# ryought/dbgphmm

Hardware: AMD Instinct MI355X
Metric: read-bases/sec through forward+backward P(R|X) (higher is better)
Workload: dtype f64; 1 GPU; cfg3: synthetic 100 kb diploid genome (1% divergence), 20x HiFi reads (p=0.001, L=1000), k=40 DBG; sparse-adaptive forward+backward+posteriors (generate_mappings); n_nodes=131694, n_edges=132357, reads_rank0=4026, bases_rank0=4000713, total_bases=4000713, spin_up_steps=12

## Files before the change

dbgphmm_amd/csrc/api.cpp:

```cpp
#include <chrono>
#include <cstdlib>
#include <cmath>
#include <cstring>

#include "phmm_internal.h"

namespace phmm {

static thread_local std::string g_error;
static thread_local hipStream_t g_stream = nullptr;
static thread_local uint64_t g_ws_limit = 0;
static thread_local CallStats g_stats;
static thread_local bool g_timing = false;

void set_error(const std::string &msg) { g_error = msg; }
int fail(int code, const std::string &msg) {
    g_error = msg;
    return code;
}
hipStream_t current_stream() { return g_stream; }
int &workset_index() {
    static thread_local int idx = 0;
    return idx;
}
// ... 40 lines not shown
    k.no_packed = flag("PHMM_NO_PACKED");
    k.packed_cpl = num("PHMM_PACKED_CPL", 0);
    k.no_exact_hinted = flag("PHMM_NO_EXACT_HINTED");
    k.no_exact_dense = flag("PHMM_NO_EXACT_DENSE");
    k.no_wide_hinted = flag("PHMM_NO_WIDE_HINTED");
    k.wide_hinted = flag("PHMM_WIDE_HINTED") && !k.no_wide_hinted;
    k.no_wide_list_bwd = flag("PHMM_NO_WIDE_LIST_BWD");
    k.wide_edge_bwd = flag("PHMM_WIDE_EDGE_BWD");
    k.wide_states_bwd = flag("PHMM_WIDE_STATES_BWD");
    k.wide_bwd_t = num("PHMM_WIDE_BWD_T", 0);
    if (k.wide_bwd_t != 128 && k.wide_bwd_t != 448) k.wide_bwd_t = 0;
    k.wide_hinted_cpb = num("PHMM_WIDE_HINTED_CPB", 0);
    if (k.wide_hinted_cpb != 1 && k.wide_hinted_cpb != 2 && k.wide_hinted_cpb != 4) k.wide_hinted_cpb = 0;
    k.no_side_worker = flag("PHMM_NO_SIDE_WORKER");
    k.no_wide_handover = flag("PHMM_NO_WIDE_HANDOVER");
    k.workers = std::max(1, std::min(MAX_WORKERS, num("PHMM_WORKERS", 1)));
    k.warm_cols = num("PHMM_WARM_COLS", 0);
    k.chunk_groups = std::max(0, num("PHMM_CHUNK_GROUPS", 0));
    k.no_keep_all = flag("PHMM_NO_KEEP_ALL");
    k.pipeline_min_groups = std::max(1, num("PHMM_PIPELINE_MIN_GROUPS", 8));
    k.no_runmax = flag("PHMM_NO_RUNMAX");
    k.force_radix = flag("PHMM_FORCE_RADIX");
    k.no_bwd_skip = flag("PHMM_NO_BWD_SKIP");
    k.serial_emit = flag("PHMM_SERIAL_EMIT");
    k.emit_high_priority = flag("PHMM_EMIT_HIGH_PRIORITY");
    k.no_dma = flag("PHMM_NO_DMA");
    k.bwd_dma = flag("PHMM_BWD_DMA");
    k.dense_streams = num("PHMM_DENSE_STREAMS", 0);
    k.dense_w = num("PHMM_DENSE_W", 0);
    k.dense_npt = num("PHMM_DENSE_NPT", 0);
    if (const char *e = std::getenv("PHMM_MEM_FRACTION")) k.mem_fraction = std::min(0.97, std::max(0.1, std::atof(e)));
    k.share_prefix = num("PHMM_SHARE_PREFIX", -1);
    if (k.share_prefix < 0 || k.share_prefix > 6) k.share_prefix = -1;
    g_knobs = k;
}

void trace(const char *tag) {
    if (!g_knobs.trace) return;
    static thread_local std::chrono::steady_clock::time_point last = std::chrono::steady_clock::now();
    (void)hipStreamSynchronize(g_stream);
    const auto now = std::chrono::steady_clock::now();
    static const auto t0 = std::chrono::steady_clock::now();
    std::fprintf(stderr, "[phmm trace] w%d @%9.2f %-28s %8.2f ms\n", workset_index(),
                 std::chrono::duration<double, std::milli>(now - t0).count(), tag,
                 std::chrono::duration<double, std::milli>(now - last).count());
    last = now;
}

uint64_t table_budget(const DevicePool &pool, uint64_t reserve) {
    if (g_ws_limit) return g_ws_limit;
    size_t fr = 0, tot = 0;
    if (hipMemGetInfo(&fr, &tot) != hipSuccess) return (uint64_t)16 << 30;
    const double frac = g_knobs.mem_fraction > 0.0 ? g_knobs.mem_fraction : 0.9;
    const double b = frac * (double)(fr + pool.owned_table_bytes()) - (double)reserve;
    return (uint64_t)std::max(b, 64.0 * 1024 * 1024);
}
uint64_t planned_budget(const DevicePool &pool) {
    if (g_ws_limit) return g_ws_limit;
    size_t fr = 0, tot = 0;
    if (hipMemGetInfo(&fr, &tot) != hipSuccess) return (uint64_t)16 << 30;
    const double frac = g_knobs.mem_fraction > 0.0 ? g_knobs.mem_fraction : 0.95;
    return (uint64_t)(frac * (double)(fr + pool.owned_bytes()));
}

static std::mutex g_pool_mu;
static DevicePool *g_pools[64] = {};
// ... 896 lines not shown
```

dbgphmm_amd/csrc/dense.hip:

```cpp
#include <algorithm>
#include <cmath>
#include <cstring>
#include <numeric>
#include <type_traits>

#include "dense_internal.h"
#include "lds_dma.h"
#include "prefix_share.h"

#ifndef PHMM_FWD_PF
#define PHMM_FWD_PF 2
#endif
#ifndef PHMM_BWD_PF
#define PHMM_BWD_PF 1
#endif
#ifndef PHMM_SMALLW_WAVES
#define PHMM_SMALLW_WAVES 3
#endif

namespace phmm {


__device__ __forceinline__ int xcd_block(int b, int nblk8) {
    int per = nblk8 >> 3;
// ... 481 lines not shown
    const int cn = a.bcols == 2 ? ((pos + 1) & 1) : (pos + 1 < a.Lc ? pos + 1 : 0);
    const int cc = a.bcols == 2 ? (pos & 1) : pos;
    const double *nm = a.Bm + ((size_t)g * a.bcols + cn) * NW;
    const double *ni = a.Bi + ((size_t)g * a.bcols + cn) * NW;
    double *om = a.Bm + ((size_t)g * a.bcols + cc) * NW;
    double *oi = a.Bi + ((size_t)g * a.bcols + cc) * NW;
    double *od = a.Bd ? a.Bd + ((size_t)g * a.bcols + cc) * NW : nullptr;

    double wgt = 0.0, wgt2 = 0.0;
    const double *fm = nullptr, *fi = nullptr, *fd = nullptr, *gm = nullptr, *gi = nullptr, *gd = nullptr;
    const bool want_post = a.want_freq || a.want_map;
    if (want_post && live) {
        const double lpf = a.logPf[g * W + r];
        if (lpf > -INFINITY) {
            if (pos >= 1) {
                const int fe = a.FE[((size_t)g * (a.Lc + 1) + (pos - 1)) * W + r];
                wgt = exp((double)(fe + Epos) * LN2 - lpf);
            }
            if (first && !sparse_tail) {
                const int fe = a.FE[((size_t)g * (a.Lc + 1) + pos) * W + r];
                wgt2 = exp((double)fe * LN2 - lpf) * lp.p_end;
            }
        }
    }
    if (want_post) {
        const size_t cprev = ((size_t)g * a.Lc + (pos > 0 ? pos - 1 : 0)) * NW;
        const size_t ccur = ((size_t)g * a.Lc + pos) * NW;
        fm = a.Fm + cprev; fi = a.Fi + cprev; fd = a.Fd + cprev;
        gm = a.Fm + ccur; gi = a.Fi + ccur; gd = a.Fd + ccur;
    }
    int rf = r;
    if (VF && want_post) {
        const uint32_t v = share_lane_of_column(a.vlane[g * W + r], pos - 1);
        const size_t vc = ((size_t)(v / SHARE_W) * a.vLc + (pos - 1)) * NW;
        fm = a.vFm + vc; fi = a.vFi + vc; fd = a.vFd + vc;
        rf = (int)(v % SHARE_W);
    }

    double vmax = 0.0, s1 = 0.0, s2 = 0.0, pmx = 0.0, pmx2 = 0.0;
    double *Pa = a.want_map ? a.Pa + (size_t)g * NW : nullptr;
    double *Pb = a.want_map ? a.Pb + (size_t)g * NW : nullptr;
    if (lb < a.nblk && compute) {
        constexpr int H = CHAIN_HOPS;
        const int kbase = lb * (a.npt * ROWS) + row * a.npt + hull_first;
        double E1 = 0.0, E2 = 0.0, E3 = 0.0, E4 = 0.0, E5 = 0.0, Q1 = 0.0, Q2 = 0.0, Q3 = 0.0, Q4 = 0.0, Q5 = 0.0, TE = 0.0;
        int nvalid = 0;
        constexpr int PFB = DMA_ ? BDMA_DEPTH : PHMM_BWD_PF;
        double nx_m[PFB], nx_i[PFB], nx_fm[PFB], nx_fi[PFB], nx_fd[PFB];
        const double *lfm = want_post ? fm : nm, *lfi = want_post ? fi : nm, *lfd = want_post ? fd : nm;
        const int jtop = hull_top < a.N - 1 - kbase ? hull_top : a.N - 1 - kbase;
        const int l64 = threadIdx.x & 63;
        const double *srcA = (l64 < 32 ? nm : ni) + 2 * (l64 & 31);
        const double *srcB = (l64 < 32 ? lfm : lfi) + 2 * (l64 & 31);
        const double *srcC = lfd + 2 * (l64 & 31);
        const uint32_t ring_base =
            DMA_ ? (uint32_t)__builtin_amdgcn_readfirstlane(
                       (int)(uint32_t)(uintptr_t)&ring[(threadIdx.x >> 6) * BDMA_DEPTH * BDMA_SLOT])
                 : 0u;
        const double *ring_w = &ring[DMA_ ? (threadIdx.x >> 6) * BDMA_DEPTH * BDMA_SLOT : 0];
        const int n1 = __any(live) ? 2 + (od ? 1 : 0) : 0;
        if (W == 64 && a.skcells) {
            const unsigned long long nlive = (unsigned long long)__popcll(__ballot(live));
            if (l64 == 0 && jtop >= 0) atomicAdd(a.skcells, nlive * (unsigned long long)(jtop + 1));
        }
        const int ns = n1 + ((a.want_map && __any(live)) ? 1 : 0) + (a.want_freq ? 2 : 0);
#pragma unroll
        for (int u = 0; u < PFB; u++) {
            int v0 = kbase + (jtop - u > 0 ? jtop - u : 0);
// ... 960 lines not shown
```

dbgphmm_amd/csrc/dense_internal.h:

```cpp
#pragma once

#include <vector>

#include "phmm_internal.h"
#include "seg_hull.h"

namespace phmm {

static constexpr double LN2 = 0.693147180559945309417232121458;
static constexpr int BLOCK = 256;

struct DenseArgs {
    int N, ng, Lc, nblk, npt;
    int g_off;
    const NodeRec *nodes;
    const uint8_t *emis;
    const double *init, *dinit, *tdinit;
    const uint32_t *fc_off;
    const FwdEntry *fc;
    const uint32_t *bc_off;
    const BwdEntry *bc;
    const uint32_t *fh_off, *bh_off;
    const HopEntry *fh, *bh;
    int hop_mode;
// ... 6 lines not shown
    unsigned long long *cmaxF;
    double *epart;
    int eall;
    double *logPf;
    double *logE;
    double *Bm, *Bi, *Bd;
    int bcols;
    int *BE;
    unsigned long long *cmaxB;
    double *bpart;
    double *logmbB, *logibB;
    double *accg;
    int want_freq;
    int nblk8;
    unsigned long long *tmaxF;
    const int *bstart;
    int want_map;
    double *Pa, *Pb;
    double *Prun;
    unsigned long long *pmax;
    const int *wf_sw;
    const uint8_t *wf_mode;
    int *wf_sub;
    int *wf_cnt;
    uint32_t *wf_node;
    double *wf_tot;
    double wf_ratio;
    double wf_ub_a, wf_ub_b;
    const uint32_t *rs_off = nullptr, *rs = nullptr;
    uint32_t *skH = nullptr;
    uint8_t *skA = nullptr;
    int nrun = 0, nseg = 0, sseg = 1;
    unsigned long long *skcells = nullptr;
    const double *vFm = nullptr, *vFi = nullptr, *vFd = nullptr;
    const uint32_t *vlane = nullptr;
    int vLc = 0, vJ = 0;
};
static constexpr int WF_CAP = 1024;


struct Plan {
    int W, ng_total, npt, nblk, nblk8;
    std::vector<uint32_t> order;
};

Plan make_plan(const phmm_model *m, const phmm_reads *reads, int forced_w);
Plan make_plan_ids(const phmm_model *m, const phmm_reads *reads, const std::vector<uint32_t> &ids);
void layout(DenseArgs &a, int W, bool full_b, void *tables, void *misc, size_t &tb, size_t &mb,
            bool backward_only = false);
void fill_model_args(DenseArgs &a, const phmm_model *m);
void host_logib(const phmm_model *m, size_t n, std::vector<double> &out);
void launch_fwd_step(int W, const DenseArgs &a, int pos);
void launch_fwd_finish(int W, const DenseArgs &a);
void launch_bwd_step(int W, const DenseArgs &a, int pos);
void launch_bwd_finish(int W, const DenseArgs &a);

struct ExactTables {
    double *f_m, *f_i, *f_d, *f_scal, *b_m, *b_i, *b_d, *b_scal;
};
void exact_dense_reads(phmm_model *m, const uint8_t *bases, const uint64_t *off, const std::vector<uint32_t> &ids, double *lf,
                       double *lb, double *freq_dev, const ExactTables *tabs, double *edge_freq_dev = nullptr,
                       double *init_freq_dev = nullptr);
bool certify_dense(int N, int len, double log2P, const int *FE, const double *log2maxF, const int *BE, const double *log2maxB,
                   double log2_p_end);
bool certify_dense_cells(int N, int len, const int *E, const double *log2max, bool backward);

}
// ... 1 lines not shown
```

dbgphmm_amd/csrc/phmm_internal.h:

```cpp
#pragma once

#include <hip/hip_runtime.h>

#include <cstdint>
#include <cstdio>
#include <memory>
#include <mutex>
#include <string>
#include <vector>

#include "../../include/phmm_amd.h"
#include "../../include/phmm_amd_states.h"
#include "../../include/phmm_amd_path.h"
#include "../../include/phmm_amd_share.h"

namespace phmm {

void set_error(const std::string &msg);
int fail(int code, const std::string &msg);

struct Error {
    int code;
    std::string msg;
};
// ... 311 lines not shown
    bool trace = false;
    bool no_lean = false;
    bool no_wide_class = false;
    bool no_packed = false;
    int packed_cpl = 0;
    bool no_exact_hinted = false;
    bool no_exact_dense = false;
    bool wide_hinted = false;
    bool no_wide_hinted = false;
    bool no_wide_list_bwd = false;
    bool wide_edge_bwd = false;
    bool wide_states_bwd = false;
    int wide_bwd_t = 0;
    int wide_hinted_cpb = 0;
    bool no_side_worker = false;
    bool no_wide_handover = false;
    int workers = 1;
    int warm_cols = 0;
    int chunk_groups = 0;
    bool no_keep_all = false;
    int pipeline_min_groups = 8;
    bool no_runmax = false;
    bool force_radix = false;
    bool serial_emit = false;
    bool emit_high_priority = false;
    bool no_dma = false;
    bool bwd_dma = false;
    bool no_bwd_skip = false;
    int dense_streams = 0;
    int dense_w = 0;
    int dense_npt = 0;
    double mem_fraction = 0.0;
    int share_prefix = -1;
};
const Knobs &knobs();
void refresh_knobs();

void model_build_host(phmm_model *m);
void model_upload(phmm_model *m);
const RunSucc &model_run_successors(phmm_model *m, int seg);

void run_dense(phmm_model *m, const phmm_reads *reads, double *out_lf, double *out_lb,
               double *out_nf);
void full_prob_sparse_backward(phmm_model *m, const phmm_reads *reads, double *out_logp, double *out_total);
void backward_sparse_tables(phmm_model *m, const uint8_t *read, uint64_t len, double *b_m, double *b_i, double *b_d,
                            double *b_scal, uint8_t *is_dense);
void run_sparse(phmm_model *m, const phmm_reads *reads, double *out_lf, double *out_lb, double *out_nf);
void run_dense_edges(phmm_model *m, const phmm_reads *reads, double *out_lf, double *out_ef, double *out_if);
struct RecPool;
void full_prob_reads_hinted(phmm_model *m, const phmm_reads *reads, const phmm_mappings *mp, uint32_t n_cand,
                            const double *init_logp, const double *trans_logp, double *out_logp,
                            double *out_total, const RecPool *pool = nullptr, const uint32_t *copy_nums = nullptr,
                            uint32_t min_copy_num = 0);
void full_prob_reads_copy_num_changes(phmm_model *m, const phmm_reads *reads, const phmm_mappings *mp,
                                      const uint32_t *base_cn, uint32_t min_cn, uint32_t n_cand, const uint64_t *chg_off,
                                      const uint32_t *chg_node, const uint32_t *chg_cn, double *out_logp,
                                      double *out_total, uint64_t *out_n_rescored);
void likelihood_refresh(phmm_likelihood *lk);
void likelihood_score_changes(phmm_likelihood *lk, uint32_t n_cand, const uint64_t *chg_off, const uint32_t *chg_node,
                              const uint32_t *chg_cn, double *out_logp, double *out_total, uint64_t *out_n_rescored,
                              bool by_group = false);
void likelihood_move(phmm_likelihood *lk, uint64_t n_chg, const uint32_t *chg_node, const uint32_t *chg_cn,
                     double *out_total, uint64_t *out_n_rescored, bool by_group = false);
void likelihood_current(const phmm_likelihood *lk, uint32_t *out_cn, double *out_logp, double *out_total);
void upload_reads(const phmm_reads *r);
void upload_mappings(const phmm_mappings *mp);
// ... 24 lines not shown
```

dbgphmm_amd/csrc/prefix_share.h:

```cpp
#pragma once

#include <cstdint>

#if defined(__HIPCC__)
#define PHMM_SHARE_FN __host__ __device__ inline
#else
#define PHMM_SHARE_FN inline
#endif

namespace phmm {

static constexpr int SHARE_MIN_J = 2, SHARE_MAX_J = 6;
static constexpr int SHARE_W = 64;
static constexpr uint64_t SHARE_MEM_DIV = 16;

PHMM_SHARE_FN uint32_t share_lanes(int J) { return 1u << (2 * J); }
PHMM_SHARE_FN uint32_t share_groups(int J) { return (share_lanes(J) + SHARE_W - 1) / SHARE_W; }
PHMM_SHARE_FN uint64_t share_table_bytes(int J, uint64_t N) {
    return (uint64_t)share_groups(J) * (uint64_t)J * N * SHARE_W * 24;
}

PHMM_SHARE_FN int64_t share_gain(int ng, int J) { return (int64_t)ng * J - (int64_t)J * (int64_t)share_groups(J); }

PHMM_SHARE_FN int share_choose_j(int ng, uint64_t N, uint64_t cap) {
    int best = 0;
    int64_t best_gain = 0;
    for (int J = SHARE_MIN_J; J <= SHARE_MAX_J; J++) {
        if (share_table_bytes(J, N) > cap) break;
        const int64_t g = share_gain(ng, J);
        if (g > best_gain) {
            best = J;
            best_gain = g;
        }
    }
    return best;
}

PHMM_SHARE_FN uint32_t share_prefix_index(const uint8_t *digit, int J) {
    uint32_t idx = 0;
    for (int i = 0; i < J; i++) idx |= (uint32_t)(digit[i] & 3u) << (2 * i);
    return idx;
}
PHMM_SHARE_FN uint32_t share_digit(uint32_t idx, int i) { return (idx >> (2 * i)) & 3u; }
PHMM_SHARE_FN uint32_t share_lane_of_column(uint32_t idx, int j) { return idx & (share_lanes(j + 1) - 1u); }

}
```

dbgphmm_amd/csrc/sparse_dyn.hip:

```cpp
#include <algorithm>
#include <cmath>
#include <cstdlib>
#include <cstring>

#include "dense_internal.h"
#include <condition_variable>
#include <deque>
#include <exception>
#include <functional>
#include <memory>
#include <mutex>
#include <thread>

#include "frontier_dev.h"
#include "prefix_share.h"
#include "sparse_dyn.h"
#include "sparse_fwd_kernel.h"
#include "wide_fwd_kernel.h"
#include "lean_fwd_kernel.h"

namespace phmm {

struct WarmArgs {
    DenseArgs d;
// ... 159 lines not shown
    if (lane == 0) {
        if (decided) {
            wa.sw[gi] = new_sw;
            if (new_sw < len) wa.cand_n[gi] = new_cn;
        }
        wa.amb[gi] = amb ? 1 : 0;
        if (amb) atomicAdd(wa.n_amb, 1);
        else if (!decided) atomicAdd(wa.undecided, 1);
        ((uint8_t *)wa.d.wf_mode)[gi] = (!decided && pos >= 1 && nsub <= 4096) ? 1 : 0;
        wa.d.wf_sub[gi] = 0;
        wa.d.wf_cnt[gi] = 0;
    }
}

struct ShareArgs {
    DenseArgs v;
    DenseArgs d;
    const uint32_t *vlane;
    int J;
};
__global__ void __launch_bounds__(BLOCK) share_copy_ctl(const ShareArgs sa, const int lanes) {
    const int gi = blockIdx.x * BLOCK + threadIdx.x;
    if (gi >= lanes || sa.d.len[gi] == 0) return;
    const int g = gi / SHARE_W, r = gi % SHARE_W;
    const uint32_t idx = sa.vlane[gi];
    for (int j = 0; j < sa.J; j++) {
        const uint32_t v = share_lane_of_column(idx, j);
        const size_t vg = v / SHARE_W, vr = v % SHARE_W;
        sa.d.FE[((size_t)g * (sa.d.Lc + 1) + j) * SHARE_W + r] = sa.v.FE[(vg * (sa.v.Lc + 1) + j) * SHARE_W + vr];
        sa.d.cmaxF[((size_t)g * sa.d.Lc + j) * SHARE_W + r] = sa.v.cmaxF[(vg * sa.v.Lc + j) * SHARE_W + vr];
        if (j + 1 < sa.J) sa.d.tmaxF[((size_t)g * sa.d.Lc + j) * SHARE_W + r] = sa.v.tmaxF[(vg * sa.v.Lc + j) * SHARE_W + vr];
    }
}
static constexpr int SHARE_ROWS = 32;
__global__ void __launch_bounds__(BLOCK) share_expand(const ShareArgs sa, const int nrange) {
    const unsigned b = blockIdx.x;
    const unsigned t = b >> 3;
    const int g = (int)(t % (unsigned)sa.d.ng);
    const int c = (int)(t / (unsigned)sa.d.ng) * 8 + (int)(b & 7u);
    if (c >= nrange) return;
    const int r = threadIdx.x & 63, w = threadIdx.x >> 6;
    const int gi = g * SHARE_W + r;
    const bool on = sa.d.len[gi] != 0;
    const uint32_t v = sa.vlane[gi];
    const size_t NW = (size_t)sa.d.N * SHARE_W;
    const size_t so = ((size_t)(v / SHARE_W) * sa.v.Lc + (sa.J - 1)) * NW + v % SHARE_W;
    const size_t dof = ((size_t)g * sa.d.Lc + (sa.J - 1)) * NW + r;
    const double *sm = sa.v.Fm + so, *si = sa.v.Fi + so;
    double *dm = sa.d.Fm + dof, *di = sa.d.Fi + dof;
    constexpr int PER = SHARE_ROWS / (BLOCK / 64);
    double vm[PER], vi[PER];
    const int k0 = c * SHARE_ROWS + w;
#pragma unroll
    for (int u = 0; u < PER; u++) {
        const int k = k0 + u * (BLOCK / 64);
        const bool ok = on && k < sa.d.N;
        vm[u] = ok ? sm[(size_t)k * SHARE_W] : 0.0;
        vi[u] = ok ? si[(size_t)k * SHARE_W] : 0.0;
    }
#pragma unroll
    for (int u = 0; u < PER; u++) {
        const int k = k0 + u * (BLOCK / 64);
        if (on && k < sa.d.N) {
            dm[(size_t)k * SHARE_W] = vm[u];
            di[(size_t)k * SHARE_W] = vi[u];
        }
    }
}

__device__ __forceinline__ int block_count(int local, int *lds_i) {
    __syncthreads();
    if (threadIdx.x == 0) *lds_i = 0;
    __syncthreads();
    local = wave_isum(local);
    if ((threadIdx.x & 63) == 0) atomicAdd(lds_i, local);
    __syncthreads();
    return *lds_i;
}

__global__ void __launch_bounds__(BLOCK) select_top400(const Top400Args a) {
    __shared__ int cnt;
    const uint32_t gi = a.need[blockIdx.x];
    const int g = (int)(gi / a.W), r = (int)(gi % a.W);
    const int col = a.sw[gi] - 1;
    const int N = a.d.N;
    const size_t NW = (size_t)N * a.W;
    const double *fm = a.d.Fm + ((size_t)g * a.d.Lc + col) * NW;
    const double *fi = a.d.Fi + ((size_t)g * a.d.Lc + col) * NW;
    const double *fd = a.d.Fd + ((size_t)g * a.d.Lc + col) * NW;
    const double tmax = __longlong_as_double((long long)a.d.tmaxF[((size_t)g * a.d.Lc + col) * a.W + r]);
    const double thr = tmax * a.ratio_lin;
    uint32_t *sn = a.sc_node + (size_t)blockIdx.x * N;
    double *stt = a.sc_tot + (size_t)blockIdx.x * N;
    if (threadIdx.x == 0) a.sc_n[blockIdx.x] = 0;
    __syncthreads();
    for (int k = threadIdx.x; k < N; k += BLOCK) {
        const size_t ix = (size_t)k * a.W + r;
        const double t = fm[ix] + fi[ix] + fd[ix];
// ... 128 lines not shown
    uint64_t min_len = UINT64_MAX;
    for (uint64_t r = 0; r < R; r++) min_len = std::min<uint64_t>(min_len, reads->off[r + 1] - reads->off[r]);
    const int map_planes = sink ? (min_len <= (uint64_t)prm.n_warmup + 2 ? 3 : 2) : 0;
    uint64_t limit_total = 0, limit_side = 0;
    {
        const uint64_t est_fpool = reads->total * 1024 + R * 65536 + (1u << 20), est_meta = reads->total * 40,
                       est_ctl = R * (uint64_t)(PHMM_MAX_ACTIVE_NODES * 12 * 5 + WF_CAP * 12 + 4096) + reads->total,
                       est_sink = sink ? reads->total * 176 + R * 131072 + (1u << 21) : 0,
                       est_sel = (uint64_t)256 * m->N * 12;
        const uint64_t est = (est_fpool + est_meta + est_ctl) * 5 / 4 + est_sink + est_sel;
        uint64_t have = m->pool->ws_out.bytes;
        for (const auto &w : m->pool->wsets) {
            have += w.misc.bytes;
            for (int k = 0; k < 16; k++)
                if (k != 4) have += w.aux[k].bytes;
        }
        const uint64_t total = planned_budget(*m->pool), fixed = std::max(est, have);
        limit_total = total > fixed + ((uint64_t)64 << 20) ? total - fixed : (uint64_t)64 << 20;
        uint64_t n_def = std::max<uint64_t>(8, R / 50);
        if (by_ratio && reads->warm_hint.size() == R) {
            n_def = 8;
            for (uint16_t h : reads->warm_hint) n_def += h >= warm_cols ? 1 : 0;
        }
        const uint64_t per_read = ((uint64_t)(prm.n_warmup + 2) * 24 + 4 * 8 + (uint64_t)map_planes * 8) * m->N;
        uint64_t lanes_def = 1;
        while (lanes_def < std::min<uint64_t>(n_def, 64)) lanes_def <<= 1;
        if (n_def > 64) lanes_def = (n_def + 63) / 64 * 64;
        limit_side = std::min<uint64_t>(limit_total / 8, lanes_def * per_read * 9 / 8);
    }
    uint64_t limit_main = limit_total - limit_side;

    struct ShareState {
        int J = 0;
        uint32_t nvl = 0;
        DenseArgs va{};
        int digit_of[256];
        double ms = 0.0;
        uint64_t launches = 0, cells = 0;
    } share;
    share_info() = ShareInfo();
    std::vector<uint32_t> short_ids;
    if (by_ratio && main_pc->plan.W == SHARE_W && knobs().share_prefix != 0) {
        const uint64_t cap = limit_main / SHARE_MEM_DIV;
        const int forced = knobs().share_prefix;
        int J = forced > 0 ? (share_table_bytes(forced, m->N) <= cap ? forced : 0)
                           : share_choose_j(main_pc->plan.ng_total, m->N, cap);
        if (J > 0 && (int64_t)J + 2 > prm.n_warmup) J = 0;
        if (J > 0 && min_len < (uint64_t)J + 2) {
            if (forced > 0) J = 0;
            else {
                for (uint64_t r = 0; r < R; r++)
                    if (reads->off[r + 1] - reads->off[r] < (uint64_t)J + 2) short_ids.push_back((uint32_t)r);
                if (short_ids.size() > std::max<uint64_t>(8, R / 50)) J = 0;
                else {
                    std::vector<uint32_t> long_ids;
                    for (uint64_t r = 0; r < R; r++)
                        if (reads->off[r + 1] - reads->off[r] >= (uint64_t)J + 2) long_ids.push_back((uint32_t)r);
                    Plan lp = make_plan_ids(m, reads, long_ids);
                    if (lp.W == SHARE_W) main_pc->plan = std::move(lp);
                    else J = 0;
                }
                if (J == 0) short_ids.clear();
            }
        }
        const auto in_main = [&](uint64_t r) { return short_ids.empty() || reads->off[r + 1] - reads->off[r] >= (uint64_t)J + 2; };
        if (J > 0) {
            std::fill(share.digit_of, share.digit_of + 256, -1);
            bool seen[256] = {};
            for (uint8_t e : m->emission) seen[e] = true;
            int nc = 0;
            for (int b = 0; b < 256; b++)
                if (seen[b] && b != (int)'n') share.digit_of[b] = nc++;
            if (nc > 4) J = 0;
            for (uint64_t r = 0; r < R && J > 0; r++)
                for (int i = 0; i < J && in_main(r); i++)
                    if (share.digit_of[reads->bases[reads->off[r] + i]] < 0) {
                        J = 0;
                        break;
                    }
        }
        if (J > 0) {
            const uint64_t vl = (uint64_t)share_groups(J) * SHARE_W;
            const uint64_t bytes = share_table_bytes(J, m->N) + vl * ((uint64_t)PHMM_MAX_ACTIVE_NODES * 12 + 64 * (J + 1)) +
                                   (uint64_t)share_groups(J) * m->N * 8 + ((uint64_t)4 << 20);
            limit_main -= std::min(bytes, limit_main / 2);
            share.J = J;
            share.nvl = share_lanes(J);
        }
    }

    auto enqueue_plan = [&](std::unique_ptr<PlanCtx> pcu, std::deque<Item> &dst) {
        PlanCtx *pc = pcu.get();
        Plan &plan = pc->plan;
        for (uint32_t rd : plan.order) pc->max_len = std::max<uint64_t>(pc->max_len, reads->off[rd + 1] - reads->off[rd]);
        if (by_ratio && reads->warm_hint.size() == reads->R)
            std::stable_sort(plan.order.begin(), plan.order.end(),
                             [&](uint32_t x, uint32_t y) { return reads->warm_hint[x] > reads->warm_hint[y]; });
        const int W = plan.W;
        const size_t NW = (size_t)m->N * W;
        pc->d_order.upload(plan.order.data(), sizeof(uint32_t) * plan.order.size());
        HIP_CHECK(hipStreamSynchronize(current_stream()));
        int target = chunk_groups;
        if (target == 0) target = n_workers > 1 ? std::max(4, (plan.ng_total + 3 * n_workers - 1) / (3 * n_workers)) : plan.ng_total;
        const uint64_t limit = (&dst == &side_queue) ? limit_side : limit_main / (uint64_t)n_workers;
        int g0 = 0;
        while (g0 < plan.ng_total) {
            int Lc = (int)std::min<int64_t>((int64_t)pc->max_len, std::min<int64_t>(prm.n_warmup + 2, pc->lc_cap));
            if (pc->may_defer && g0 == 0 && n_workers == 1) {
                auto cost = [&](int lc) { return (size_t)lc * NW * 24 + 4 * NW * 8 + (sink ? (size_t)map_planes * NW * 8 + (size_t)plan.nblk8 * BLOCK * 8 : 0); };
                const int lc_full = (int)std::min<int64_t>((int64_t)pc->max_len, prm.n_warmup + 2);
                if ((uint64_t)plan.ng_total * cost(lc_full) <= limit && !knobs().no_keep_all) Lc = lc_full;
                else
                    for (int cut = 0; cut <= 2 && Lc - cut >= 8; cut++)
                        if ((uint64_t)plan.ng_total * cost(Lc - cut) <= limit) {
                            Lc -= cut;
                            break;
                        }
            }
            const size_t per_group = (size_t)Lc * NW * 24 + 4 * NW * 8 + (sink ? (size_t)map_planes * NW * 8 + (size_t)plan.nblk8 * BLOCK * 8 : 0);
            int ngc = (int)std::min<uint64_t>(plan.ng_total - g0, std::max<uint64_t>(1, limit / std::max<size_t>(per_group, 1)));
            ngc = std::min(ngc, std::max(1, target));
            int Lfull = 1;
            for (size_t slot = (size_t)g0 * W; slot < std::min<size_t>(plan.order.size(), (size_t)(g0 + ngc) * W); slot++) {
                const uint32_t rd = plan.order[slot];
                Lfull = std::max(Lfull, (int)(reads->off[rd + 1] - reads->off[rd]));
            }
            dst.push_back(Item{pc, g0, ngc, std::min(Lc, Lfull), Lfull});
            g0 += ngc;
        }
        plans.push_back(std::move(pcu));
    };

    std::function<void()> start_side_worker;
    auto run_chunk = [&](const Item &it) {
        hipStream_t s = current_stream();
        CallStats &st = stats();
        DevBuf &warm = m->wset().aux[0];
        DevBuf &fpool = m->wset().aux[1], &fpool_meta = m->wset().aux[2];
        const Plan &plan = it.pc->plan;
        const DevBuf &d_order = it.pc->d_order;
        const int W = plan.W;
        const uint64_t R = plan.order.size();
        const int g0 = it.g0, ngc = it.ngc, Lc = it.Lc, Lfull = it.Lfull;
// ... 55 lines not shown
        }
        std::vector<double> hib;
        host_logib(m, (size_t)Lc, hib);
        std::vector<int> hlc(hl);
        for (auto &v : hlc) v = std::min(v, Lc);
        {
            StageArgs sa{};
            sa.bases = reads->d_bases.as<uint8_t>();
            sa.off = reads->d_off.as<uint64_t>();
            sa.order = d_order.as<uint32_t>() + (size_t)g0 * W;
            sa.n_slots = (uint32_t)(R - std::min<uint64_t>(R, (uint64_t)g0 * W));
            sa.W = W;
            sa.Lc = Lc;
            sa.Lfull = Lfull;
            sa.out_dense = (uint8_t *)a.bases;
            sa.out_full = (uint8_t *)(wp + o_bases);
            const unsigned per_group = (unsigned)Lfull * W;
            hipLaunchKernelGGL(stage_bases, dim3((per_group + BLOCK - 1) / BLOCK, ngc), dim3(BLOCK), 0, s, sa);
            HIP_CHECK(hipGetLastError());
        }
        HIP_CHECK(hipMemcpyAsync((void *)a.len, hlc.data(), hlc.size() * sizeof(int), hipMemcpyHostToDevice, s));
        HIP_CHECK(hipMemcpyAsync((void *)a.logib, hib.data(), hib.size() * sizeof(double), hipMemcpyHostToDevice, s));
        std::vector<uint32_t> hvl(shared ? (size_t)lanes : 0, 0u);
        if (shared) {
            for (int gi = 0; gi < lanes; gi++) {
                const size_t slot = (size_t)g0 * W + gi;
                if (slot >= R) continue;
                const uint8_t *rb = reads->bases.data() + reads->off[plan.order[slot]];
                uint8_t dg[SHARE_MAX_J];
                for (int i = 0; i < share.J; i++) dg[i] = (uint8_t)share.digit_of[rb[i]];
                hvl[gi] = share_prefix_index(dg, share.J);
            }
            HIP_CHECK(hipMemcpyAsync(wp + o_vlane, hvl.data(), sizeof(uint32_t) * lanes, hipMemcpyHostToDevice, s));
            a.vFm = share.va.Fm;
            a.vFi = share.va.Fi;
            a.vFd = share.va.Fd;
            a.vlane = (const uint32_t *)(wp + o_vlane);
            a.vLc = share.va.Lc;
            a.vJ = share.J;
        }
        HIP_CHECK(hipStreamSynchronize(s));

        WarmArgs wa{};
        wa.d = a;
        wa.sw = (int *)(wp + o_sw);
        wa.cnt = (int *)(wp + o_cnt);
        wa.cand_n = (int *)(wp + o_cn);
        wa.undecided = (int *)(wp + o_und);
        wa.n_amb = wa.undecided + 1;
        wa.amb = (int *)(wp + o_amb);
        a.wf_sw = by_ratio ? wa.sw : nullptr;
        a.wf_mode = (const uint8_t *)(wp + o_mode);
        a.wf_sub = (int *)(wp + o_wsub);
        a.wf_cnt = (int *)(wp + o_wcnt);
        a.wf_node = (uint32_t *)(wp + o_wnode);
        a.wf_tot = (double *)(wp + o_wtot);
        a.wf_ratio = std::exp(-prm.active_node_max_ratio);
        a.wf_ub_a = m->wf_ub_a;
        a.wf_ub_b = m->wf_ub_b;
        wa.d = a;
        wa.cand_node = (uint32_t *)(wp + o_cnode);
        wa.cand_tot = (double *)(wp + o_ctot);
        wa.ratio_lin = std::exp(-prm.active_node_max_ratio);
        wa.n_warmup = (int)prm.n_warmup;
        wa.threshold = (int)prm.warmup_threshold;

        trace("staging+upload");
        int pos = 0;
        const bool st_on = W == 64 && (it.pc->may_defer || !by_ratio);
        LaunchTimer lt(timing_enabled() && st_on);
        std::unique_lock<std::mutex> dense_lock(dense_token, std::defer_lock);
        const bool use_token = it.pc->may_defer || !by_ratio;
        if (use_token) dense_lock.lock();
        if (shared) {
            ShareArgs sa{share.va, a, a.vlane, share.J};
            const int nrange = (int)((m->N + SHARE_ROWS - 1) / SHARE_ROWS), nrange8 = (nrange + 7) / 8 * 8;
            lt.begin();
            hipLaunchKernelGGL(share_copy_ctl, dim3((lanes + BLOCK - 1) / BLOCK), dim3(BLOCK), 0, s, sa, lanes);
            hipLaunchKernelGGL(share_expand, dim3((unsigned)nrange8 * (unsigned)ngc), dim3(BLOCK), 0, s, sa, nrange);
            lt.end();
            HIP_CHECK(hipGetLastError());
            pos = share.J;
        }
        if (!by_ratio) {
            const int last = std::min<int>((int)prm.n_warmup, Lc);
            for (pos = 0; pos <= last; pos++) {
                lt.begin();
                launch_fwd_step(W, a, pos);
                lt.end();
                if (st_on) st.launches[0]++;
            }
            std::vector<int> fsw(lanes);
            for (int gi = 0; gi < lanes; gi++) fsw[gi] = std::min<int>((int)prm.n_warmup, hl[gi]);
            HIP_CHECK(hipMemcpyAsync(wa.sw, fsw.data(), sizeof(int) * lanes, hipMemcpyHostToDevice, s));
            HIP_CHECK(hipStreamSynchronize(s));
        }
        for (; by_ratio; pos++) {
            lt.begin();
            launch_fwd_step(W, a, pos);
            lt.end();
            if (st_on) st.launches[0]++;
            HIP_CHECK(hipMemsetAsync(wa.undecided, 0, sizeof(int) * 2, s));
            hipLaunchKernelGGL(warm_decide_fused, dim3((lanes + BLOCK / 64 - 1) / (BLOCK / 64)), dim3(BLOCK), 0, s, wa, pos,
                               lanes, W);
            int und[2] = {0, 0};
            HIP_CHECK(hipMemcpyAsync(und, wa.undecided, sizeof(int) * 2, hipMemcpyDeviceToHost, s));
            HIP_CHECK(hipStreamSynchronize(s));
            if (und[1] > 0) {
                launch_col_count_w(W, wa, pos - 1);
                hipLaunchKernelGGL(warm_decide, dim3((lanes + BLOCK - 1) / BLOCK), dim3(BLOCK), 0, s, wa, pos, lanes);
                HIP_CHECK(hipMemcpyAsync(und, wa.undecided, sizeof(int), hipMemcpyDeviceToHost, s));
                HIP_CHECK(hipStreamSynchronize(s));
// ... 308 lines not shown
            {
                std::unique_lock<std::mutex> lk(mu);
                cv.wait(lk, [&] { return !queue.empty() || active == 0 || first_error; });
                if (first_error || queue.empty()) break;
                it = queue.front();
                queue.pop_front();
                active++;
            }
            try {
                run_chunk(it);
            } catch (...) {
                std::lock_guard<std::mutex> lk(mu);
                if (!first_error) first_error = std::current_exception();
            }
            {
                std::lock_guard<std::mutex> lk(mu);
                active--;
            }
            cv.notify_all();
        }
    };

    auto build_share = [&](const Plan &mplan) {
        hipStream_t s = current_stream();
        const int J = share.J;
        const int nvg = (int)share_groups(J), vl = nvg * SHARE_W;
        DevBuf &vtab = m->pool->wsets[0].aux[22], &vmisc = m->pool->wsets[0].aux[23];
        DenseArgs va{};
        fill_model_args(va, m);
        va.nblk = mplan.nblk;
        va.nblk8 = mplan.nblk8;
        va.npt = mplan.npt;
        va.ng = nvg;
        va.Lc = J;
        size_t tb = 0, mb = 0;
        layout(va, SHARE_W, false, nullptr, nullptr, tb, mb);
        vtab.reserve((size_t)share_table_bytes(J, m->N) + 1024);
        size_t cb = (mb + 255) / 256 * 256;
        auto carve = [&](size_t bytes) {
            cb = (cb + 255) / 256 * 256;
            const size_t o = cb;
            cb += bytes;
            return o;
        };
        const size_t o_sw = carve(sizeof(int) * vl), o_cnt = carve(sizeof(int) * vl), o_cn = carve(sizeof(int) * vl),
                     o_und = carve(sizeof(int) * 2), o_amb = carve(sizeof(int) * vl),
                     o_cnode = carve(sizeof(uint32_t) * (size_t)vl * PHMM_MAX_ACTIVE_NODES),
                     o_ctot = carve(sizeof(double) * (size_t)vl * PHMM_MAX_ACTIVE_NODES);
        vmisc.reserve(cb);
        layout(va, SHARE_W, false, vtab.p, vmisc.p, tb, mb);
        char *cp = (char *)vmisc.p;
        HIP_CHECK(hipMemsetAsync(cp, 0, o_cnode, s));
        HIP_CHECK(hipMemsetAsync(cp + o_sw, 0xff, sizeof(int) * vl, s));
        HIP_CHECK(hipMemsetAsync(cp + o_amb, 0x01, sizeof(int) * vl, s));
        uint8_t code_of[4] = {0xfe, 0xfe, 0xfe, 0xfe};
        for (int b = 0; b < 256; b++)
            if (share.digit_of[b] >= 0) code_of[share.digit_of[b]] = (uint8_t)b;
        std::vector<uint8_t> hb((size_t)nvg * J * SHARE_W, 0xff);
        std::vector<int> hlen((size_t)vl, 0);
        for (uint32_t v = 0; v < share.nvl; v++) {
            hlen[v] = J;
            for (int i = 0; i < J; i++) hb[((size_t)(v / SHARE_W) * J + i) * SHARE_W + v % SHARE_W] = code_of[share_digit(v, i)];
        }
        std::vector<double> hib;
        host_logib(m, (size_t)J, hib);
        HIP_CHECK(hipMemcpyAsync((void *)va.bases, hb.data(), hb.size(), hipMemcpyHostToDevice, s));
        HIP_CHECK(hipMemcpyAsync((void *)va.len, hlen.data(), hlen.size() * sizeof(int), hipMemcpyHostToDevice, s));
        HIP_CHECK(hipMemcpyAsync((void *)va.logib, hib.data(), hib.size() * sizeof(double), hipMemcpyHostToDevice, s));
        LaunchTimer lt(timing_enabled());
        for (int pos = 0; pos < J; pos++) {
            lt.begin();
            launch_fwd_step(SHARE_W, va, pos);
            lt.end();
        }
        WarmArgs vwa{};
        vwa.d = va;
        vwa.sw = (int *)(cp + o_sw);
        vwa.cnt = (int *)(cp + o_cnt);
        vwa.cand_n = (int *)(cp + o_cn);
        vwa.undecided = (int *)(cp + o_und);
        vwa.n_amb = vwa.undecided + 1;
        vwa.amb = (int *)(cp + o_amb);
        vwa.cand_node = (uint32_t *)(cp + o_cnode);
        vwa.cand_tot = (double *)(cp + o_ctot);
        vwa.ratio_lin = std::exp(-prm.active_node_max_ratio);
        vwa.n_warmup = (int)prm.n_warmup;
        vwa.threshold = (int)prm.warmup_threshold;
        for (int col = 0; col + 1 < J; col++) {
            launch_col_count_w(SHARE_W, vwa, col);
            hipLaunchKernelGGL(warm_decide, dim3((vl + BLOCK - 1) / BLOCK), dim3(BLOCK), 0, s, vwa, col + 1, vl);
        }
        HIP_CHECK(hipGetLastError());
        std::vector<int> hsw((size_t)vl, -1);
        HIP_CHECK(hipMemcpyAsync(hsw.data(), vwa.sw, sizeof(int) * vl, hipMemcpyDeviceToHost, s));
        HIP_CHECK(hipStreamSynchronize(s));
        share.ms = lt.total_ms();
        share.launches = (uint64_t)J;
        share.cells = (uint64_t)share.nvl * (uint64_t)J * m->N;
        share.va = va;
        for (uint32_t v = 0; v < share.nvl; v++)
            if (hsw[v] >= 0) {
                if (knobs().trace) std::fprintf(stderr, "      prefix sharing declined: virtual lane %u leaves the warm-up at position %d\n", v, hsw[v]);
                share.J = 0;
                break;
            }
        trace("prefix sharing: virtual plan");
    };

    {
        const int min_groups = knobs().pipeline_min_groups;
        if (main_pc->plan.ng_total < min_groups) n_workers = 1;
        const Plan &mplan = main_pc->plan;
        enqueue_plan(std::move(main_pc), queue);
        for (const Item &it : queue)
            if (share.J + 2 > it.Lc) share.J = 0;
        if (share.J > 0) build_share(mplan);
        if (share.J > 0) share_info() = ShareInfo{share.J, (uint64_t)share.nvl};
    }
    const int n_threads = (int)std::min<size_t>((size_t)n_workers, queue.size());
    if (!short_ids.empty()) {
        std::unique_ptr<PlanCtx> pc(new PlanCtx{make_plan_ids(m, reads, short_ids), (int64_t)prm.n_warmup + 2, false, {}});
        const size_t side_group = ((size_t)(prm.n_warmup + 2) * 24 + 4 * 8 + (size_t)map_planes * 8) * m->N * pc->plan.W;
        std::lock_guard<std::mutex> lk(mu);
        if (n_threads <= 1 && side_on && side_group <= limit_side) {
            enqueue_plan(std::move(pc), side_queue);
            side_started = true;
            start_side_worker();
        } else {
            enqueue_plan(std::move(pc), queue);
        }
    }
// ... 69 lines not shown
```

Measured before the change: 33.51 million bases/s.

## Widen prefix-sharing table progressively so early columns compute only distinct prefixes

Adds a "widening" prefix-sharing mode that is on by default. Column j of the virtual prefix table is computed only for the 4^(j+1) distinct prefixes instead of all 4^J lanes. A tiled LDS-staged expand kernel copies column states into the wider group set between steps and also replaces the per-group strided expand into the main tables. This cuts redundant forward work and table memory for the shared prefix, so a larger J can fit in the memory cap. The cost is more complex pointer aliasing, extra copy kernels per column and risk of indexing errors.

New measurement: 27.86 million bases/s. 0.831x the previous value.

```diff
diff --git a/dbgphmm_amd/csrc/api.cpp b/dbgphmm_amd/csrc/api.cpp
--- a/dbgphmm_amd/csrc/api.cpp
+++ b/dbgphmm_amd/csrc/api.cpp
@@ -96,6 +96,8 @@
     if (const char *e = std::getenv("PHMM_MEM_FRACTION")) k.mem_fraction = std::min(0.97, std::max(0.1, std::atof(e)));
     k.share_prefix = num("PHMM_SHARE_PREFIX", -1);
     if (k.share_prefix < 0 || k.share_prefix > 6) k.share_prefix = -1;
+    k.share_widen = num("PHMM_SHARE_WIDEN", -1);
+    if (k.share_widen != 0 && k.share_widen != 1) k.share_widen = -1;
     g_knobs = k;
 }
 
diff --git a/dbgphmm_amd/csrc/dense.hip b/dbgphmm_amd/csrc/dense.hip
--- a/dbgphmm_amd/csrc/dense.hip
+++ b/dbgphmm_amd/csrc/dense.hip
@@ -537,8 +537,8 @@
     int rf = r;
     if (VF && want_post) {
         const uint32_t v = share_lane_of_column(a.vlane[g * W + r], pos - 1);
-        const size_t vc = ((size_t)(v / SHARE_W) * a.vLc + (pos - 1)) * NW;
-        fm = a.vFm + vc; fi = a.vFi + vc; fd = a.vFd + vc;
+        fm = a.vcol[pos - 1] + (size_t)(v / SHARE_W) * a.vLc * NW;
+        fi = fm + a.voI; fd = fm + a.voD;
         rf = (int)(v % SHARE_W);
     }
 
diff --git a/dbgphmm_amd/csrc/dense_internal.h b/dbgphmm_amd/csrc/dense_internal.h
--- a/dbgphmm_amd/csrc/dense_internal.h
+++ b/dbgphmm_amd/csrc/dense_internal.h
@@ -62,7 +62,8 @@
     uint8_t *skA = nullptr;
     int nrun = 0, nseg = 0, sseg = 1;
     unsigned long long *skcells = nullptr;
-    const double *vFm = nullptr, *vFi = nullptr, *vFd = nullptr;
+    const double *vcol[6] = {nullptr, nullptr, nullptr, nullptr, nullptr, nullptr};
+    long long voI = 0, voD = 0;
     const uint32_t *vlane = nullptr;
     int vLc = 0, vJ = 0;
 };
diff --git a/dbgphmm_amd/csrc/phmm_internal.h b/dbgphmm_amd/csrc/phmm_internal.h
--- a/dbgphmm_amd/csrc/phmm_internal.h
+++ b/dbgphmm_amd/csrc/phmm_internal.h
@@ -367,6 +367,7 @@
     int dense_npt = 0;
     double mem_fraction = 0.0;
     int share_prefix = -1;
+    int share_widen = -1;
 };
 const Knobs &knobs();
 void refresh_knobs();
diff --git a/dbgphmm_amd/csrc/prefix_share.h b/dbgphmm_amd/csrc/prefix_share.h
--- a/dbgphmm_amd/csrc/prefix_share.h
+++ b/dbgphmm_amd/csrc/prefix_share.h
@@ -36,6 +36,33 @@
     return best;
 }
 
+static constexpr int SHARE_WIDEN_SLOTS = 5;
+PHMM_SHARE_FN uint32_t share_widen_lanes(int j) { return 1u << (2 * (j + 1)); }
+PHMM_SHARE_FN uint32_t share_widen_groups(int j) { return (share_widen_lanes(j) + SHARE_W - 1) / SHARE_W; }
+PHMM_SHARE_FN uint32_t share_widen_cost(int J) {
+    uint32_t c = 0;
+    for (int j = 0; j < J; j++) c += share_widen_groups(j);
+    return c;
+}
+PHMM_SHARE_FN int share_widen_slots(int J) { return J > SHARE_WIDEN_SLOTS ? J : SHARE_WIDEN_SLOTS; }
+PHMM_SHARE_FN uint64_t share_widen_table_bytes(int J, uint64_t N) {
+    return (uint64_t)share_widen_cost(J) * (uint64_t)share_widen_slots(J) * N * SHARE_W * 8;
+}
+PHMM_SHARE_FN int64_t share_widen_gain(int ng, int J) { return (int64_t)ng * J - (int64_t)share_widen_cost(J); }
+PHMM_SHARE_FN int share_widen_choose_j(int ng, uint64_t N, uint64_t cap) {
+    int best = 0;
+    int64_t best_gain = 0;
+    for (int J = SHARE_MIN_J; J <= SHARE_MAX_J; J++) {
+        if (share_widen_table_bytes(J, N) > cap) break;
+        const int64_t g = share_widen_gain(ng, J);
+        if (g > best_gain) {
+            best = J;
+            best_gain = g;
+        }
+    }
+    return best;
+}
+
 PHMM_SHARE_FN uint32_t share_prefix_index(const uint8_t *digit, int J) {
     uint32_t idx = 0;
     for (int i = 0; i < J; i++) idx |= (uint32_t)(digit[i] & 3u) << (2 * i);
diff --git a/dbgphmm_amd/csrc/sparse_dyn.hip b/dbgphmm_amd/csrc/sparse_dyn.hip
--- a/dbgphmm_amd/csrc/sparse_dyn.hip
+++ b/dbgphmm_amd/csrc/sparse_dyn.hip
@@ -215,38 +215,59 @@
         if (j + 1 < sa.J) sa.d.tmaxF[((size_t)g * sa.d.Lc + j) * SHARE_W + r] = sa.v.tmaxF[(vg * sa.v.Lc + j) * SHARE_W + vr];
     }
 }
-static constexpr int SHARE_ROWS = 32;
-__global__ void __launch_bounds__(BLOCK) share_expand(const ShareArgs sa, const int nrange) {
-    const unsigned b = blockIdx.x;
-    const unsigned t = b >> 3;
-    const int g = (int)(t % (unsigned)sa.d.ng);
-    const int c = (int)(t / (unsigned)sa.d.ng) * 8 + (int)(b & 7u);
-    if (c >= nrange) return;
+__global__ void __launch_bounds__(BLOCK) share_widen_ctl(const DenseArgs v, const int j, const int lanes, const uint32_t mask) {
+    const uint32_t gi = blockIdx.x * BLOCK + threadIdx.x, s = gi & mask;
+    if (gi >= (uint32_t)lanes || s == gi) return;
+    const size_t g = gi / SHARE_W, r = gi % SHARE_W, sg = s / SHARE_W, sr = s % SHARE_W;
+    v.FE[(g * (v.Lc + 1) + j) * SHARE_W + r] = v.FE[(sg * (v.Lc + 1) + j) * SHARE_W + sr];
+    v.cmaxF[(g * v.Lc + j) * SHARE_W + r] = v.cmaxF[(sg * v.Lc + j) * SHARE_W + sr];
+}
+struct ShareCopy {
+    const double *sm;
+    double *dm;
+    long long soI, doI;
+    size_t sstride, dstride;
+    const uint32_t *vlane;
+    const int *len;
+    uint32_t mask;
+    int ng, N;
+};
+static constexpr uint32_t SHARE_TILE_BYTES = 16u << 10;
+static inline uint32_t share_tile_bytes() { return SHARE_TILE_BYTES; }
+static inline int share_src_groups(uint32_t mask) { return (int)((mask + SHARE_W) / SHARE_W); }
+static inline int share_tile_rows(uint32_t mask) {
+    const uint32_t row_bytes = (uint32_t)share_src_groups(mask) * SHARE_W * 8u;
+    return (int)std::max(1u, std::min(32u, share_tile_bytes() / row_bytes));
+}
+__global__ void __launch_bounds__(BLOCK) share_expand(const ShareCopy sc, const int rows) {
+    extern __shared__ double share_tile[];
+    const int SG = (int)((sc.mask + SHARE_W) / SHARE_W), SL = SG * SHARE_W;
+    const int k0 = (int)blockIdx.x * rows;
     const int r = threadIdx.x & 63, w = threadIdx.x >> 6;
-    const int gi = g * SHARE_W + r;
-    const bool on = sa.d.len[gi] != 0;
-    const uint32_t v = sa.vlane[gi];
-    const size_t NW = (size_t)sa.d.N * SHARE_W;
-    const size_t so = ((size_t)(v / SHARE_W) * sa.v.Lc + (sa.J - 1)) * NW + v % SHARE_W;
-    const size_t dof = ((size_t)g * sa.d.Lc + (sa.J - 1)) * NW + r;
-    const double *sm = sa.v.Fm + so, *si = sa.v.Fi + so;
-    double *dm = sa.d.Fm + dof, *di = sa.d.Fi + dof;
-    constexpr int PER = SHARE_ROWS / (BLOCK / 64);
-    double vm[PER], vi[PER];
-    const int k0 = c * SHARE_ROWS + w;
-#pragma unroll
-    for (int u = 0; u < PER; u++) {
-        const int k = k0 + u * (BLOCK / 64);
-        const bool ok = on && k < sa.d.N;
-        vm[u] = ok ? sm[(size_t)k * SHARE_W] : 0.0;
-        vi[u] = ok ? si[(size_t)k * SHARE_W] : 0.0;
-    }
-#pragma unroll
-    for (int u = 0; u < PER; u++) {
-        const int k = k0 + u * (BLOCK / 64);
-        if (on && k < sa.d.N) {
-            dm[(size_t)k * SHARE_W] = vm[u];
-            di[(size_t)k * SHARE_W] = vi[u];
+    const double *src = blockIdx.y ? sc.sm + sc.soI : sc.sm;
+#pragma unroll 4
+    for (int it = w; it < rows * SG; it += BLOCK / 64) {
+        const int sg = it % SG, row = it / SG;
+        const int k = k0 + row;
+        if (k < sc.N) share_tile[(size_t)row * SL + sg * SHARE_W + r] = src[(size_t)sg * sc.sstride + (size_t)k * SHARE_W + r];
+    }
+    __syncthreads();
+    const auto lane_of = [&](int g, bool &on) {
+        const int gi = g * SHARE_W + r;
+        on = sc.len == nullptr || sc.len[gi] != 0;
+        return (sc.vlane ? sc.vlane[gi] : (uint32_t)gi) & sc.mask;
+    };
+    bool on_next = false;
+    uint32_t v_next = w < sc.ng ? lane_of(w, on_next) : 0u;
+    for (int g = w; g < sc.ng; g += BLOCK / 64) {
+        const uint32_t v = v_next;
+        const bool on = on_next;
+        if (g + BLOCK / 64 < sc.ng) v_next = lane_of(g + BLOCK / 64, on_next);
+        double *dst = (blockIdx.y ? sc.dm + sc.doI : sc.dm) + (size_t)g * sc.dstride + r;
+        for (int row = 0; row < rows; row++) {
+            const int k = k0 + row;
+            if (k >= sc.N) break;
+            if (on) dst[(size_t)k * SHARE_W] = share_tile[(size_t)row * SL + v];
         }
     }
 }
@@ -441,8 +462,11 @@
 
     struct ShareState {
         int J = 0;
+        bool widen = false;
         uint32_t nvl = 0;
         DenseArgs va{};
+        const double *vcol[SHARE_MAX_J] = {};
+        long long voI = 0, voD = 0;
         int digit_of[256];
         double ms = 0.0;
         uint64_t launches = 0, cells = 0;
@@ -452,8 +476,25 @@
     if (by_ratio && main_pc->plan.W == SHARE_W && knobs().share_prefix != 0) {
         const uint64_t cap = limit_main / SHARE_MEM_DIV;
         const int forced = knobs().share_prefix;
-        int J = forced > 0 ? (share_table_bytes(forced, m->N) <= cap ? forced : 0)
-                           : share_choose_j(main_pc->plan.ng_total, m->N, cap);
+        const bool widen = knobs().share_widen == 1 || (knobs().share_widen < 0 && forced <= 0);
+        const auto table_bytes = [&](int j) { return widen ? share_widen_table_bytes(j, m->N) : share_table_bytes(j, m->N); };
+        const auto share_bytes = [&](int j) {
+            const uint64_t vl = (uint64_t)share_groups(j) * SHARE_W;
+            return table_bytes(j) + vl * ((uint64_t)PHMM_MAX_ACTIVE_NODES * 12 + 64 * (j + 1)) + (uint64_t)share_groups(j) * m->N * 8 +
+                   ((uint64_t)4 << 20);
+        };
+        int J = forced > 0 ? (table_bytes(forced) <= cap ? forced : 0)
+                           : (widen ? share_widen_choose_j(main_pc->plan.ng_total, m->N, cap)
+                                    : share_choose_j(main_pc->plan.ng_total, m->N, cap));
+        if (widen && forced <= 0 && (knobs().workers == 1 || main_pc->plan.ng_total < knobs().pipeline_min_groups)) {
+            const Plan &pl = main_pc->plan;
+            const size_t NW = (size_t)m->N * pl.W;
+            const int64_t lc = std::min<int64_t>((int64_t)reads->max_len, std::min<int64_t>(prm.n_warmup + 2, main_pc->lc_cap));
+            const uint64_t need = (uint64_t)pl.ng_total * ((uint64_t)lc * NW * 24 + 4 * NW * 8 +
+                                                           (sink ? (uint64_t)map_planes * NW * 8 + (uint64_t)pl.nblk8 * BLOCK * 8 : 0));
+            if (need <= limit_main)
+                while (J > 0 && share_bytes(J) > limit_main - need) J = share_widen_choose_j(pl.ng_total, m->N, std::min(cap, table_bytes(J) - 1));
+        }
         if (J > 0 && (int64_t)J + 2 > prm.n_warmup) J = 0;
         if (J > 0 && min_len < (uint64_t)J + 2) {
             if (forced > 0) J = 0;
@@ -489,11 +530,9 @@
                     }
         }
         if (J > 0) {
-            const uint64_t vl = (uint64_t)share_groups(J) * SHARE_W;
-            const uint64_t bytes = share_table_bytes(J, m->N) + vl * ((uint64_t)PHMM_MAX_ACTIVE_NODES * 12 + 64 * (J + 1)) +
-                                   (uint64_t)share_groups(J) * m->N * 8 + ((uint64_t)4 << 20);
-            limit_main -= std::min(bytes, limit_main / 2);
+            limit_main -= std::min(share_bytes(J), limit_main / 2);
             share.J = J;
+            share.widen = widen;
             share.nvl = share_lanes(J);
         }
     }
@@ -518,6 +557,9 @@
             if (pc->may_defer && g0 == 0 && n_workers == 1) {
                 auto cost = [&](int lc) { return (size_t)lc * NW * 24 + 4 * NW * 8 + (sink ? (size_t)map_planes * NW * 8 + (size_t)plan.nblk8 * BLOCK * 8 : 0); };
                 const int lc_full = (int)std::min<int64_t>((int64_t)pc->max_len, prm.n_warmup + 2);
+                if (knobs().trace)
+                    std::fprintf(stderr, "      main plan: %d groups, %d kept columns take %.2f GB of %.2f GB\n", plan.ng_total, Lc,
+                                 (double)plan.ng_total * (double)cost(Lc) / 1e9, (double)limit / 1e9);
                 if ((uint64_t)plan.ng_total * cost(lc_full) <= limit && !knobs().no_keep_all) Lc = lc_full;
                 else
                     for (int cut = 0; cut <= 2 && Lc - cut >= 8; cut++)
@@ -639,9 +681,9 @@
                 hvl[gi] = share_prefix_index(dg, share.J);
             }
             HIP_CHECK(hipMemcpyAsync(wp + o_vlane, hvl.data(), sizeof(uint32_t) * lanes, hipMemcpyHostToDevice, s));
-            a.vFm = share.va.Fm;
-            a.vFi = share.va.Fi;
-            a.vFd = share.va.Fd;
+            for (int j = 0; j < share.J; j++) a.vcol[j] = share.vcol[j];
+            a.voI = share.voI;
+            a.voD = share.voD;
             a.vlane = (const uint32_t *)(wp + o_vlane);
             a.vLc = share.va.Lc;
             a.vJ = share.J;
@@ -681,10 +723,24 @@
         if (use_token) dense_lock.lock();
         if (shared) {
             ShareArgs sa{share.va, a, a.vlane, share.J};
-            const int nrange = (int)((m->N + SHARE_ROWS - 1) / SHARE_ROWS), nrange8 = (nrange + 7) / 8 * 8;
+            const size_t NW = (size_t)m->N * SHARE_W;
+            ShareCopy sc{};
+            sc.sm = share.vcol[share.J - 1];
+            sc.soI = share.voI;
+            sc.sstride = (size_t)share.va.Lc * NW;
+            sc.dm = a.Fm + (size_t)(share.J - 1) * NW;
+            sc.doI = a.Fi - a.Fm;
+            sc.dstride = (size_t)a.Lc * NW;
+            sc.vlane = a.vlane;
+            sc.len = a.len;
+            sc.mask = share.nvl - 1u;
+            sc.ng = ngc;
+            sc.N = (int)m->N;
+            const int rows = share_tile_rows(sc.mask);
             lt.begin();
             hipLaunchKernelGGL(share_copy_ctl, dim3((lanes + BLOCK - 1) / BLOCK), dim3(BLOCK), 0, s, sa, lanes);
-            hipLaunchKernelGGL(share_expand, dim3((unsigned)nrange8 * (unsigned)ngc), dim3(BLOCK), 0, s, sa, nrange);
+            hipLaunchKernelGGL(share_expand, dim3((unsigned)((m->N + rows - 1) / rows), 2), dim3(BLOCK),
+                               (size_t)rows * share_src_groups(sc.mask) * SHARE_W * sizeof(double), s, sc, rows);
             lt.end();
             HIP_CHECK(hipGetLastError());
             pos = share.J;
@@ -1059,10 +1115,17 @@
         va.nblk8 = mplan.nblk8;
         va.npt = mplan.npt;
         va.ng = nvg;
-        va.Lc = J;
+        const bool widen = share.widen;
+        const int Lc = widen ? share_widen_slots(J) : J;
+        const size_t NW = (size_t)m->N * SHARE_W;
+        const auto groups_of = [&](int j) { return widen ? (int)share_widen_groups(j) : nvg; };
+        va.Lc = Lc;
         size_t tb = 0, mb = 0;
         layout(va, SHARE_W, false, nullptr, nullptr, tb, mb);
-        vtab.reserve((size_t)share_table_bytes(J, m->N) + 1024);
+        vtab.reserve((size_t)(widen ? share_widen_table_bytes(J, m->N) : share_table_bytes(J, m->N)) + 1024);
+        if (knobs().trace)
+            std::fprintf(stderr, "      prefix sharing: J %d, %s, %d group-columns, tables %.2f GB\n", J, widen ? "widening" : "uniform",
+                         widen ? (int)share_widen_cost(J) : J * nvg, (double)vtab.bytes / 1e9);
         size_t cb = (mb + 255) / 256 * 256;
         auto carve = [&](size_t bytes) {
             cb = (cb + 255) / 256 * 256;
@@ -1083,11 +1146,28 @@
         uint8_t code_of[4] = {0xfe, 0xfe, 0xfe, 0xfe};
         for (int b = 0; b < 256; b++)
             if (share.digit_of[b] >= 0) code_of[share.digit_of[b]] = (uint8_t)b;
-        std::vector<uint8_t> hb((size_t)nvg * J * SHARE_W, 0xff);
+        std::vector<uint8_t> hb((size_t)nvg * Lc * SHARE_W, 0xff);
         std::vector<int> hlen((size_t)vl, 0);
         for (uint32_t v = 0; v < share.nvl; v++) {
             hlen[v] = J;
-            for (int i = 0; i < J; i++) hb[((size_t)(v / SHARE_W) * J + i) * SHARE_W + v % SHARE_W] = code_of[share_digit(v, i)];
+            for (int i = 0; i < J; i++) hb[((size_t)(v / SHARE_W) * Lc + i) * SHARE_W + v % SHARE_W] = code_of[share_digit(v, i)];
+        }
+        DenseArgs la[SHARE_MAX_J];
+        {
+            double *tj = (double *)vtab.p;
+            for (int j = 0; j < J; j++) {
+                la[j] = va;
+                la[j].ng = groups_of(j);
+                if (widen) {
+                    la[j].Fm = tj + (ptrdiff_t)(1 - j) * (ptrdiff_t)NW;
+                    la[j].Fi = tj + (ptrdiff_t)(3 - j) * (ptrdiff_t)NW;
+                    la[j].Fd = tj + (ptrdiff_t)(5 - j) * (ptrdiff_t)NW;
+                    tj += (size_t)la[j].ng * Lc * NW;
+                }
+            }
+            for (int j = 0; j < J; j++) share.vcol[j] = j + 1 < J ? la[j + 1].Fm + (size_t)j * NW : la[j].Fm + (size_t)j * NW;
+            share.voI = widen ? 2 * (long long)NW : (long long)(va.Fi - va.Fm);
+            share.voD = widen ? 4 * (long long)NW : (long long)(va.Fd - va.Fm);
         }
         std::vector<double> hib;
         host_logib(m, (size_t)J, hib);
@@ -1097,7 +1177,22 @@
         LaunchTimer lt(timing_enabled());
         for (int pos = 0; pos < J; pos++) {
             lt.begin();
-            launch_fwd_step(SHARE_W, va, pos);
+            if (widen && pos >= 1) {
+                const int ngd = la[pos].ng, ld = ngd * SHARE_W;
+                ShareCopy sc{};
+                sc.sm = la[pos - 1].Fm + (size_t)(pos - 1) * NW;
+                sc.dm = la[pos].Fm + (size_t)(pos - 1) * NW;
+                sc.soI = sc.doI = 2 * (long long)NW;
+                sc.sstride = sc.dstride = (size_t)Lc * NW;
+                sc.mask = share_widen_lanes(pos - 1) - 1u;
+                sc.ng = ngd;
+                sc.N = (int)m->N;
+                hipLaunchKernelGGL(share_widen_ctl, dim3((ld + BLOCK - 1) / BLOCK), dim3(BLOCK), 0, s, va, pos - 1, ld, sc.mask);
+                const int rows = share_tile_rows(sc.mask);
+                hipLaunchKernelGGL(share_expand, dim3((unsigned)((m->N + rows - 1) / rows), 2), dim3(BLOCK),
+                                   (size_t)rows * share_src_groups(sc.mask) * SHARE_W * sizeof(double), s, sc, rows);
+            }
+            launch_fwd_step(SHARE_W, la[pos], pos);
             lt.end();
         }
         WarmArgs vwa{};
@@ -1114,8 +1209,11 @@
         vwa.n_warmup = (int)prm.n_warmup;
         vwa.threshold = (int)prm.warmup_threshold;
         for (int col = 0; col + 1 < J; col++) {
+            const int cl = groups_of(col) * SHARE_W;
+            vwa.d = la[col + 1];
+            vwa.d.ng = groups_of(col);
             launch_col_count_w(SHARE_W, vwa, col);
-            hipLaunchKernelGGL(warm_decide, dim3((vl + BLOCK - 1) / BLOCK), dim3(BLOCK), 0, s, vwa, col + 1, vl);
+            hipLaunchKernelGGL(warm_decide, dim3((cl + BLOCK - 1) / BLOCK), dim3(BLOCK), 0, s, vwa, col + 1, cl);
         }
         HIP_CHECK(hipGetLastError());
         std::vector<int> hsw((size_t)vl, -1);
@@ -1123,7 +1221,8 @@
         HIP_CHECK(hipStreamSynchronize(s));
         share.ms = lt.total_ms();
         share.launches = (uint64_t)J;
-        share.cells = (uint64_t)share.nvl * (uint64_t)J * m->N;
+        share.cells = 0;
+        for (int j = 0; j < J; j++) share.cells += (uint64_t)(widen ? share_widen_lanes(j) : share.nvl) * m->N;
         share.va = va;
         for (uint32_t v = 0; v < share.nvl; v++)
             if (hsw[v] >= 0) {
```
